# freshman97/LinTransUNet

Hardware: AMD Instinct MI355X
Metric: 128^3 CT patches/sec (fwd+bwd) (higher is better)
Workload: dtype bf16; 1 GPU; MaskTransUnet train step (fwd + 5-level loss + bwd), 128^3 single-channel patches, 2 per GPU, dropout 0.3, random-init weights; global_batch=2, parallelism=dp1, side_stream_concurrent=True, allreduce=none (1 rank)

## Files before the change

### lintransunet_amd/csrc/linattn.hip

```cpp
#include "common.h"

#define DK 32
#define TOK 32
#define PART_STRIDE (64 + 1024)
#ifndef LA_TR_PAD
#define LA_TR_PAD 32
#endif

__device__ __forceinline__ float xhalf_sum(float v) { return xhalf_combine<LtuAdd>(v); }
__device__ __forceinline__ float xhalf_max(float v) { return xhalf_combine<LtuMax>(v); }

__device__ __forceinline__ bf16x8 pack8(const float* v) {
  bf16x8 r;
#pragma unroll
  for (int e = 0; e < 8; ++e) r[e] = (__bf16)v[e];
  return r;
}
template <typename T>
struct IsBf16 { static constexpr bool value = false; };
template <>
struct IsBf16<bf16_t> { static constexpr bool value = true; };

template <typename T>
struct GVec;
template <>
struct GVec<float> {
  static constexpr int W = 4;
  typedef float4 reg;
  static __device__ __forceinline__ reg load(const float* p) { return *reinterpret_cast<const float4*>(p); }
  static __device__ __forceinline__ reg zero() { return make_float4(0.f, 0.f, 0.f, 0.f); }
  static __device__ __forceinline__ void to_lds(float* dst, reg v) { *reinterpret_cast<float4*>(dst) = v; }
  static __device__ __forceinline__ void from_lds(float* gdst, const float* src) {
    *reinterpret_cast<float4*>(gdst) = *reinterpret_cast<const float4*>(src);
  }
  static __device__ __forceinline__ reg pack_lds(const float* src) { return *reinterpret_cast<const float4*>(src); }
  static __device__ __forceinline__ void store_g(float* gdst, reg v) { *reinterpret_cast<float4*>(gdst) = v; }
};
template <>
struct GVec<bf16_t> {
  static constexpr int W = 8;
  typedef uint4 reg;
  static __device__ __forceinline__ reg load(const bf16_t* p) { return *reinterpret_cast<const uint4*>(p); }
  static __device__ __forceinline__ reg zero() { return make_uint4(0u, 0u, 0u, 0u); }
  static __device__ __forceinline__ void to_lds(float* dst, reg v) {
    float4 a, b;
    a.x = __uint_as_float(v.x << 16); a.y = __uint_as_float(v.x & 0xffff0000u);
    a.z = __uint_as_float(v.y << 16); a.w = __uint_as_float(v.y & 0xffff0000u);
    b.x = __uint_as_float(v.z << 16); b.y = __uint_as_float(v.z & 0xffff0000u);
    b.z = __uint_as_float(v.w << 16); b.w = __uint_as_float(v.w & 0xffff0000u);
    *reinterpret_cast<float4*>(dst) = a;
    *reinterpret_cast<float4*>(dst + 4) = b;
  }
  static __device__ __forceinline__ void from_lds(bf16_t* gdst, const float* src) {
    const float4 a = *reinterpret_cast<const float4*>(src), b = *reinterpret_cast<const float4*>(src + 4);
    uint4 v;
    v.x = pack_bf16x2(a.x, a.y);
    v.y = pack_bf16x2(a.z, a.w);
    v.z = pack_bf16x2(b.x, b.y);
    v.w = pack_bf16x2(b.z, b.w);
    *reinterpret_cast<uint4*>(gdst) = v;
  }
  static __device__ __forceinline__ reg pack_lds(const float* src) {
    const float4 a = *reinterpret_cast<const float4*>(src), b = *reinterpret_cast<const float4*>(src + 4);
    return make_uint4(pack_bf16x2(a.x, a.y), pack_bf16x2(a.z, a.w), pack_bf16x2(b.x, b.y), pack_bf16x2(b.z, b.w));
  }
  static __device__ __forceinline__ void store_g(bf16_t* gdst, reg v) { *reinterpret_cast<uint4*>(gdst) = v; }
};

template <typename T, int D, int ROWE, int LDSROW>
struct RowTile {
  static constexpr int NTHR = 2 * D;
  static constexpr int W = GVec<T>::W;
  static constexpr int VPR = ROWE / W;
  static constexpr int NV = (TOK * VPR + NTHR - 1) / NTHR;
  typename GVec<T>::reg r[NV];
  __device__ __forceinline__ void load(const T* gbase, long long gstride, int goff, int n0, int n_end, int tid) {
#pragma unroll
    for (int p = 0; p < NV; ++p) {
      const int idx = tid + p * NTHR;
      const int t = idx / VPR, c = (idx % VPR) * W;
      r[p] = (idx < TOK * VPR && n0 + t < n_end) ? GVec<T>::load(gbase + (long long)(n0 + t) * gstride + goff + c) : GVec<T>::zero();
    }
  }
  __device__ __forceinline__ void store(float* lds, int tid) const {
#pragma unroll
    for (int p = 0; p < NV; ++p) {
      const int idx = tid + p * NTHR;
      const int t = idx / VPR, c = (idx % VPR) * W;
      if (idx < TOK * VPR) GVec<T>::to_lds(lds + t * LDSROW + c, r[p]);
    }
  }
  __device__ __forceinline__ void store_raw(uint16_t* lds, int tid) const {
#pragma unroll
    for (int p = 0; p < NV; ++p) {
      const int idx = tid + p * NTHR;
      const int t = idx / VPR, c = (idx % VPR) * W;
      if (idx < TOK * VPR) *reinterpret_cast<typename GVec<T>::reg*>(lds + t * LDSROW + c) = r[p];
    }
  }
};

typedef __attribute__((ext_vector_type(4))) short la_s16x4;
typedef __attribute__((address_space(3))) la_s16x4 la_lds_s16x4;
__device__ __forceinline__ int tr_lane_offset(int lane, int pitch) {
  const int gq = lane >> 4, tq = (lane >> 2) & 3, tp = lane & 3;
  return (8 * (gq >> 1) + tq) * pitch + 16 * (gq & 1) + 4 * tp;
}
__device__ __forceinline__ bf16x8 tr_frag(const uint16_t* p, int pitch) {
  union { struct { la_s16x4 l, h; } s; bf16x8 v; } u;
  u.s.l = __builtin_amdgcn_ds_read_tr16_b64_v4i16((la_lds_s16x4*)p);
  u.s.h = __builtin_amdgcn_ds_read_tr16_b64_v4i16((la_lds_s16x4*)(p + 4 * pitch));
  return u.v;
}

template <typename T, int D>
__global__ void __launch_bounds__(2 * D) linattn_kv_partial(const T* __restrict__ qkv, float* __restrict__ part, int N,
                                                           int tokens_per_split) {
  constexpr int H = D / DK, ROW = 2 * D;
  constexpr int PITCH = ROW + LA_TR_PAD;
  constexpr int SMEM_FLOATS = IsBf16<T>::value ? (2 * TOK * PITCH) / 2 : TOK * ROW;
  __shared__ __attribute__((aligned(16))) float smem[SMEM_FLOATS];
  const int b = blockIdx.y, sp = blockIdx.x, nsplit = gridDim.x;
  const int tid = threadIdx.x, lane = tid & 63, wave = tid >> 6;
  const int li = lane & 31, lh = lane >> 5;
  const int n_begin = sp * tokens_per_split;
  const int n_end = min(N, n_begin + tokens_per_split);
  const T* base = qkv + (long long)b * N * 3 * D;

  float m_run = -INFINITY, s_run = 0.f;
  f32x16 acc;
#pragma unroll
  for (int r = 0; r < 16; ++r) acc[r] = 0.f;

  if constexpr (IsBf16<T>::value) {
    uint16_t* sm = reinterpret_cast<uint16_t*>(smem);
    RowTile<T, D, ROW, PITCH> tile;
    const int koff = tr_lane_offset(lane, PITCH) + wave * DK, voff = koff + D;
    tile.load(base, 3 * D, D, n_begin, n_end, tid);
    tile.store_raw(sm, tid);
    __syncthreads();
    int buf = 0;
    for (int n0 = n_begin; n0 < n_end; n0 += TOK) {
      const bool more = n0 + TOK < n_end;
      if (more) tile.load(base, 3 * D, D, n0 + TOK, n_end, tid);
      const uint16_t* S = sm + buf * (TOK * PITCH);
      bf16x8 kf[2], vf[2];
#pragma unroll
      for (int u = 0; u < 2; ++u) {
        kf[u] = tr_frag(S + 16 * u * PITCH + koff, PITCH);
        vf[u] = tr_frag(S + 16 * u * PITCH + voff, PITCH);
      }
      const int ntok = min(TOK, n_end - n0);
      float kx[2][8];
      float mt = -INFINITY;
#pragma unroll
      for (int u = 0; u < 2; ++u)
#pragma unroll
        for (int e = 0; e < 8; ++e) {
          kx[u][e] = (float)kf[u][e];
          if (16 * u + 8 * lh + e < ntok) mt = fmaxf(mt, kx[u][e]);
        }
      mt = xhalf_max(mt);
      const float m_new = fmaxf(m_run, mt);
      const float alpha = __expf(m_run - m_new);
      m_run = m_new;
      s_run *= alpha;
#pragma unroll
      for (int r = 0; r < 16; ++r) acc[r] *= alpha;
#pragma unroll
      for (int u = 0; u < 2; ++u) {
        float pe[8];
#pragma unroll
        for (int e = 0; e < 8; ++e) {
          pe[e] = 16 * u + 8 * lh + e < ntok ? __expf(kx[u][e] - m_new) : 0.f;
          s_run += pe[e];
        }
        acc = __builtin_amdgcn_mfma_f32_32x32x16_bf16(vf[u], pack8(pe), acc, 0, 0, 0);
      }
      if (more) tile.store_raw(sm + (buf ^ 1) * (TOK * PITCH), tid);
      __syncthreads();
      buf ^= 1;
    }
  } else {
  RowTile<T, D, ROW, ROW> tile;
  tile.load(base, 3 * D, D, n_begin, n_end, tid);
  for (int n0 = n_begin; n0 < n_end; n0 += TOK) {
    __syncthreads();
    tile.store(smem, tid);
    __syncthreads();
    if (n0 + TOK < n_end) tile.load(base, 3 * D, D, n0 + TOK, n_end, tid);
    const int ntok = min(TOK, n_end - n0);
    const float* ks = smem + wave * DK;
    const float* vs = smem + D + wave * DK;
    float mt = -INFINITY;
#pragma unroll 4
    for (int t = lh; t < TOK; t += 2)
      if (t < ntok) mt = fmaxf(mt, ks[t * ROW + li]);
    mt = xhalf_max(mt);
    const float m_new = fmaxf(m_run, mt);
    const float alpha = __expf(m_run - m_new);
    m_run = m_new;
    s_run *= alpha;
#pragma unroll
    for (int r = 0; r < 16; ++r) acc[r] *= alpha;
    if constexpr (IsBf16<T>::value) {
#pragma unroll
      for (int u = 0; u < 2; ++u) {
        float pe[8], ve[8];
#pragma unroll
        for (int e = 0; e < 8; ++e) {
          const int t = 16 * u + 8 * lh + e;
          pe[e] = 0.f; ve[e] = 0.f;
          if (t < ntok) {
            pe[e] = __expf(ks[t * ROW + li] - m_new);
            ve[e] = vs[t * ROW + li];
          }
          s_run += pe[e];
        }
        acc = __builtin_amdgcn_mfma_f32_32x32x16_bf16(pack8(ve), pack8(pe), acc, 0, 0, 0);
      }
    } else {
#pragma unroll
      for (int t0 = 0; t0 < TOK; t0 += 2) {
        const int t = t0 + lh;
        float p = 0.f, vv = 0.f;
        if (t < ntok) {
          p = __expf(ks[t * ROW + li] - m_new);
          vv = vs[t * ROW + li];
        }
        s_run += p;
        acc = __builtin_amdgcn_mfma_f32_32x32x2f32(vv, p, acc, 0, 0, 0);
      }
    }
  }
  }
  const float s_tot = xhalf_sum(s_run);
  float* out = part + (((long long)b * nsplit + sp) * H + wave) * PART_STRIDE;
  if (lh == 0) {
    out[li] = m_run;
    out[32 + li] = s_tot;
  }
#pragma unroll
  for (int r = 0; r < 16; ++r) {
    const int j = (r & 3) + 8 * (r >> 2) + 4 * lh;
    out[64 + j * 32 + li] = acc[r];
  }
}

#define KVC_GROUP 16
__global__ void __launch_bounds__(1024) linattn_kv_combine(const float* __restrict__ part, int nsplit, int group,
                                                           float* __restrict__ part2, float* __restrict__ stats,
                                                           float* __restrict__ ctx, int H, int final) {
  const int bh = blockIdx.y, b = bh / H, h = bh % H, g = blockIdx.x;
  const int i = threadIdx.x & 31, j = threadIdx.x >> 5;
  const float* p0 = part + ((long long)b * nsplit * H + h) * PART_STRIDE;
  const long long sstride = (long long)H * PART_STRIDE;
  const int s0 = g * group, s1 = min(nsplit, s0 + group);
  float mv[KVC_GROUP];
#pragma unroll
  for (int q = 0; q < KVC_GROUP; ++q) mv[q] = s0 + q < s1 ? p0[(s0 + q) * sstride + i] : -INFINITY;
  float m = mv[0];
#pragma unroll
  for (int q = 1; q < KVC_GROUP; ++q) m = fmaxf(m, mv[q]);
  float sv[KVC_GROUP], av[KVC_GROUP];
#pragma unroll
  for (int q = 0; q < KVC_GROUP; ++q) {
    const float* p = p0 + (s0 + q) * sstride;
    sv[q] = s0 + q < s1 ? p[32 + i] : 0.f;
    av[q] = s0 + q < s1 ? p[64 + j * 32 + i] : 0.f;
  }
  float ssum = 0.f, a = 0.f;
#pragma unroll
  for (int q = 0; q < KVC_GROUP; ++q) {
    const float f = __expf(mv[q] - m);
    ssum += sv[q] * f;
    a += av[q] * f;
  }
  if (final) {
    ctx[(long long)bh * 1024 + i * 32 + j] = a / ssum;
    if (j == 0) {
      stats[bh * 64 + i] = m;
      stats[bh * 64 + 32 + i] = ssum;
    }
  } else {
    float* o = part2 + (((long long)b * gridDim.x + g) * H + h) * PART_STRIDE;
    o[64 + j * 32 + i] = a;
    if (j == 0) {
      o[i] = m;
      o[32 + i] = ssum;
    }
  }
}

template <int NB>
__global__ void __launch_bounds__(256) linattn_kv_combine1(const float* __restrict__ part, int nsplit, float* __restrict__ stats,
                                                           float* __restrict__ ctx, int H) {
  extern __shared__ __attribute__((aligned(16))) float fs[];
  __shared__ float red[8][32];
  __shared__ float4 red4[7][32];
  const int bh = blockIdx.y, b = bh / H, h = bh % H;
  const float* p0 = part + ((long long)b * nsplit * H + h) * PART_STRIDE;
  const long long sstride = (long long)H * PART_STRIDE;
  const int l = threadIdx.x & 31, grp = threadIdx.x >> 5;
  const bool fast = nsplit <= 8 * NB;
  float m = -INFINITY, ss = 0.f;
  const int e0 = blockIdx.x * 128 + l * 4, c0 = e0 & 31;
  float4 a = make_float4(0.f, 0.f, 0.f, 0.f);
  if (fast) {
    float pm[NB], ps[NB];
#pragma unroll
    for (int k = 0; k < NB; ++k) {
      const int sp = grp + 8 * k, sc = sp < nsplit ? sp : 0;
      pm[k] = p0[sc * sstride + l];
      ps[k] = p0[sc * sstride + 32 + l];
    }
#pragma unroll
    for (int k = 0; k < NB; ++k)
      if (grp + 8 * k < nsplit) m = fmaxf(m, pm[k]);
    red[grp][l] = m;
    __syncthreads();
#pragma unroll
    for (int q = 0; q < 8; ++q) m = fmaxf(m, red[q][l]);
    __syncthreads();
    float4 v[NB];
#pragma unroll
    for (int k = 0; k < NB; ++k) {
      const int sp = grp + 8 * k, sc = sp < nsplit ? sp : 0;
      v[k] = *reinterpret_cast<const float4*>(p0 + sc * sstride + 64 + e0);
    }
#pragma unroll
    for (int k = 0; k < NB; ++k) {
      const int sp = grp + 8 * k;
      if (sp < nsplit) {
        const float f = __expf(pm[k] - m);
        fs[sp * 32 + l] = f;
        ss += ps[k] * f;
      }
    }
    red[grp][l] = ss;
    __syncthreads();
    ss = 0.f;
#pragma unroll
    for (int q = 0; q < 8; ++q) ss += red[q][l];
#pragma unroll
    for (int k = 0; k < NB; ++k) {
      const int sp = grp + 8 * k;
      if (sp < nsplit) {
        const float4 f = *reinterpret_cast<const float4*>(fs + sp * 32 + c0);
        a.x += v[k].x * f.x; a.y += v[k].y * f.y; a.z += v[k].z * f.z; a.w += v[k].w * f.w;
      }
    }
  } else {
#pragma unroll 8
    for (int s = grp; s < nsplit; s += 8) m = fmaxf(m, p0[s * sstride + l]);
    red[grp][l] = m;
    __syncthreads();
#pragma unroll
    for (int q = 0; q < 8; ++q) m = fmaxf(m, red[q][l]);
    __syncthreads();
#pragma unroll 8
    for (int s = grp; s < nsplit; s += 8) {
      const float f = __expf(p0[s * sstride + l] - m);
      fs[s * 32 + l] = f;
      ss += p0[s * sstride + 32 + l] * f;
    }
    red[grp][l] = ss;
    __syncthreads();
    ss = 0.f;
#pragma unroll
    for (int q = 0; q < 8; ++q) ss += red[q][l];
#pragma unroll 8
    for (int s = grp; s < nsplit; s += 8) {
      const float4 v = *reinterpret_cast<const float4*>(p0 + s * sstride + 64 + e0);
      const float4 f = *reinterpret_cast<const float4*>(fs + s * 32 + c0);
      a.x += v.x * f.x; a.y += v.y * f.y; a.z += v.z * f.z; a.w += v.w * f.w;
    }
  }
  if (grp > 0) red4[grp - 1][l] = a;
  __shared__ float scol[32];
  if (grp == 0) scol[l] = ss;
  __syncthreads();
  if (grp != 0) return;
#pragma unroll
  for (int q = 0; q < 7; ++q) {
    const float4 v = red4[q][l];
    a.x += v.x; a.y += v.y; a.z += v.z; a.w += v.w;
  }
  const int j = e0 >> 5;
  float* o = ctx + (long long)bh * 1024 + j;
  o[c0 * 32] = a.x / scol[c0]; o[(c0 + 1) * 32] = a.y / scol[c0 + 1]; o[(c0 + 2) * 32] = a.z / scol[c0 + 2]; o[(c0 + 3) * 32] = a.w / scol[c0 + 3];
  if (blockIdx.x == 0) {
    stats[bh * 64 + l] = m;
    stats[bh * 64 + 32 + l] = ss;
  }
}

template <typename T, int D>
__global__ void __launch_bounds__(2 * D) linattn_apply(const T* __restrict__ qkv, const float* __restrict__ ctx, T* __restrict__ out,
                                                      float* __restrict__ qstat, int N, int tokb) {
  constexpr int H = D / DK, LDQ = D + 4, NTHR = 2 * D, W = GVec<T>::W;
  __shared__ __attribute__((aligned(16))) float smem[TOK * LDQ];
  const int b = blockIdx.y;
  const int tid = threadIdx.x, lane = tid & 63, wave = tid >> 6;
  const int li = lane & 31, lh = lane >> 5;
  float cb[16];
  const float* cx = ctx + ((long long)b * H + wave) * 1024;
#pragma unroll
  for (int s = 0; s < 16; ++s) cb[s] = cx[(16 * lh + s) * 32 + li];
  const bf16x8 cbb[2] = {pack8(cb), pack8(cb + 8)};
  const float rs = 0.17677669529663688110f;
  const T* base = qkv + (long long)b * N * 3 * D;

  const int n_begin = blockIdx.x * tokb;
  const int n_end = min(N, n_begin + tokb);
  RowTile<T, D, D, LDQ> tile;
  tile.load(base, 3 * D, 0, n_begin, n_end, tid);
  for (int n0 = n_begin; n0 < n_end; n0 += TOK) {
    __syncthreads();
    tile.store(smem, tid);
    __syncthreads();
    if (n0 + TOK < n_end) tile.load(base, 3 * D, 0, n0 + TOK, n_end, tid);
    float a[16];
    const float* qrow = &smem[li * LDQ + wave * DK + 16 * lh];
#pragma unroll
    for (int q4 = 0; q4 < 4; ++q4) {
      const float4 v = *reinterpret_cast<const float4*>(qrow + 4 * q4);
      a[4 * q4] = v.x; a[4 * q4 + 1] = v.y; a[4 * q4 + 2] = v.z; a[4 * q4 + 3] = v.w;
    }
    float mx = -INFINITY;
#pragma unroll
    for (int s = 0; s < 16; ++s) mx = fmaxf(mx, a[s]);
    mx = xhalf_max(mx);
    float sum = 0.f;
#pragma unroll
    for (int s = 0; s < 16; ++s) {
      a[s] = __expf(a[s] - mx);
      sum += a[s];
    }
    sum = xhalf_sum(sum);
    const float inv = rs / sum;
    if (lh == 0 && n0 + li < n_end) {
      float* qs = qstat + (((long long)b * N + n0 + li) * H + wave) * 2;
      qs[0] = mx;
      qs[1] = inv;
    }
    f32x16 acc;
#pragma unroll
    for (int r = 0; r < 16; ++r) acc[r] = 0.f;
    if constexpr (IsBf16<T>::value) {
#pragma unroll
      for (int s = 0; s < 16; ++s) a[s] *= inv;
      acc = __builtin_amdgcn_mfma_f32_32x32x16_bf16(pack8(a), cbb[0], acc, 0, 0, 0);
      acc = __builtin_amdgcn_mfma_f32_32x32x16_bf16(pack8(a + 8), cbb[1], acc, 0, 0, 0);
    } else {
#pragma unroll
      for (int s = 0; s < 16; ++s) acc = __builtin_amdgcn_mfma_f32_32x32x2f32(a[s] * inv, cb[s], acc, 0, 0, 0);
    }
    __syncthreads();
#pragma unroll
    for (int r = 0; r < 16; ++r) {
      const int t = (r & 3) + 8 * (r >> 2) + 4 * lh;
      smem[t * LDQ + wave * DK + li] = acc[r];
    }
    __syncthreads();
    constexpr int VPR = D / W;
#pragma unroll
    for (int p = 0; p < (TOK * VPR + NTHR - 1) / NTHR; ++p) {
      const int idx = tid + p * NTHR;
      const int t = idx / VPR, c = (idx % VPR) * W;
      if (idx < TOK * VPR && n0 + t < n_end) GVec<T>::from_lds(out + ((long long)b * N + n0 + t) * D + c, &smem[t * LDQ + c]);
    }
  }
}

#define LAW_HEADS 4
#define LAW_LD (LAW_HEADS * DK + 8)

template <int D>
__global__ void __launch_bounds__(256) linattn_apply_rows(const uint16_t* __restrict__ qkv, const float* __restrict__ ctx,
                                                         uint16_t* __restrict__ out, float* __restrict__ qstat, int N, int tiles_per_wave) {
  constexpr int H = D / DK, CG = H / LAW_HEADS;
  __shared__ __attribute__((aligned(16))) uint16_t smem[4 * TOK * LAW_LD];
  const int lane = threadIdx.x & 63, wave = threadIdx.x >> 6;
  const int li = lane & 31, lh = lane >> 5;
  uint16_t* tile = smem + wave * TOK * LAW_LD;
  const int b = blockIdx.y;
  const int gw = blockIdx.x * 4 + wave;
  const int cg = gw % CG;
  const int n_begin = (gw / CG) * tiles_per_wave * TOK;
  const int n_end = min(N, n_begin + tiles_per_wave * TOK);
  if (n_begin >= N) return;
  bf16x8 ca[LAW_HEADS][2];
#pragma unroll
  for (int hh = 0; hh < LAW_HEADS; ++hh) {
    const float* cx = ctx + ((long long)b * H + cg * LAW_HEADS + hh) * 1024;
#pragma unroll
    for (int u = 0; u < 2; ++u) {
      float t[8];
#pragma unroll
      for (int e = 0; e < 8; ++e) t[e] = cx[(16 * lh + 8 * u + e) * 32 + li];
      ca[hh][u] = pack8(t);
    }
  }
  const float rs = 0.17677669529663688110f;
  const int cr = lane >> 4, cc = (lane & 15) * 8;
  const uint16_t* qb = qkv + (long long)b * N * 3 * D + cg * (LAW_HEADS * DK) + cc;
  uint16_t* ob = out + (long long)b * N * D + cg * (LAW_HEADS * DK) + cc;
  uint4 nx[8];
  auto fetch = [&](int n0) {
#pragma unroll
    for (int p = 0; p < 8; ++p) {
      const int n = n0 + 4 * p + cr;
      nx[p] = make_uint4(0u, 0u, 0u, 0u);
      if (n < n_end) nx[p] = *reinterpret_cast<const uint4*>(qb + (long long)n * 3 * D);
    }
  };
  fetch(n_begin);
  for (int n0 = n_begin; n0 < n_end; n0 += TOK) {
#pragma unroll
    for (int p = 0; p < 8; ++p) *reinterpret_cast<uint4*>(tile + (4 * p + cr) * LAW_LD + cc) = nx[p];
    if (n0 + TOK < n_end) fetch(n0 + TOK);
    float2 st[LAW_HEADS];
#pragma unroll
    for (int hh = 0; hh < LAW_HEADS; ++hh) {
      const uint16_t* qr = tile + li * LAW_LD + hh * DK + 16 * lh;
      const uint4 v0 = *reinterpret_cast<const uint4*>(qr), v1 = *reinterpret_cast<const uint4*>(qr + 8);
      const uint32_t w[8] = {v0.x, v0.y, v0.z, v0.w, v1.x, v1.y, v1.z, v1.w};
      float a[16];
#pragma unroll
      for (int k = 0; k < 8; ++k) {
        a[2 * k] = __uint_as_float(w[k] << 16);
        a[2 * k + 1] = __uint_as_float(w[k] & 0xffff0000u);
      }
      float mx = a[0];
#pragma unroll
      for (int s = 1; s < 16; ++s) mx = fmaxf(mx, a[s]);
      mx = xhalf_max(mx);
      float sum = 0.f;
#pragma unroll
      for (int s = 0; s < 16; ++s) {
        a[s] = __expf(a[s] - mx);
        sum += a[s];
      }
      sum = xhalf_sum(sum);
      const float inv = rs / sum;
      st[hh] = make_float2(mx, inv);
#pragma unroll
      for (int s = 0; s < 16; ++s) a[s] *= inv;
      f32x16 acc;
#pragma unroll
      for (int r = 0; r < 16; ++r) acc[r] = 0.f;
      acc = __builtin_amdgcn_mfma_f32_32x32x16_bf16(ca[hh][0], pack8(a), acc, 0, 0, 0);
      acc = __builtin_amdgcn_mfma_f32_32x32x16_bf16(ca[hh][1], pack8(a + 8), acc, 0, 0, 0);
#pragma unroll
      for (int q = 0; q < 4; ++q) {
        uint2 v;
        v.x = pack_bf16x2(acc[4 * q], acc[4 * q + 1]);
        v.y = pack_bf16x2(acc[4 * q + 2], acc[4 * q + 3]);
        *reinterpret_cast<uint2*>(tile + li * LAW_LD + hh * DK + 8 * q + 4 * lh) = v;
      }
    }
    if (lh == 0 && n0 + li < n_end) {
      float4* qs = reinterpret_cast<float4*>(qstat + (((long long)b * N + n0 + li) * H + cg * LAW_HEADS) * 2);
      qs[0] = make_float4(st[0].x, st[0].y, st[1].x, st[1].y);
      qs[1] = make_float4(st[2].x, st[2].y, st[3].x, st[3].y);
    }
#pragma unroll
    for (int p = 0; p < 8; ++p) {
      const int n = n0 + 4 * p + cr;
      const uint4 v = *reinterpret_cast<const uint4*>(tile + (4 * p + cr) * LAW_LD + cc);
      if (n < n_end) *reinterpret_cast<uint4*>(ob + (long long)n * D) = v;
    }
  }
}

template <typename T, int D>
__global__ void __launch_bounds__(2 * D) linattn_dctx_partial(const T* __restrict__ qkv, const T* __restrict__ dout,
                                                             const float* __restrict__ qstat, float* __restrict__ part, int N,
                                                             int tokens_per_split) {
  constexpr int H = D / DK;
  extern __shared__ __attribute__((aligned(16))) float smem[];
  float* sq = smem;
  float* sg = smem + TOK * D;
  float* st = smem + 2 * TOK * D;
  const int b = blockIdx.y, sp = blockIdx.x, nsplit = gridDim.x;
  const int tid = threadIdx.x, lane = tid & 63, wave = tid >> 6;
  const int li = lane & 31, lh = lane >> 5;
  const int n_begin = sp * tokens_per_split;
  const int n_end = min(N, n_begin + tokens_per_split);
  const T* qb = qkv + (long long)b * N * 3 * D;
  const T* gb = dout + (long long)b * N * D;
  f32x16 acc;
#pragma unroll
  for (int r = 0; r < 16; ++r) acc[r] = 0.f;
  RowTile<T, D, D, D> tq, tg;
  static_assert(TOK * H * 2 <= 2 * D, "one statistics float per thread");
  auto load_stat = [&](int n0) {
    return (tid < TOK * H * 2 && n0 + tid / (H * 2) < n_end) ? qstat[((long long)b * N + n0) * H * 2 + tid] : 0.f;
  };
  if constexpr (IsBf16<T>::value) {
    constexpr int PQ = D + LA_TR_PAD;
    uint16_t* sm = reinterpret_cast<uint16_t*>(smem);
    float* stf = reinterpret_cast<float*>(sm + 4 * TOK * PQ);
    RowTile<T, D, D, PQ> bq, bg;
    const int off = tr_lane_offset(lane, PQ) + wave * DK;
    bq.load(qb, 3 * D, 0, n_begin, n_end, tid);
    bg.load(gb, D, 0, n_begin, n_end, tid);
    float stn = load_stat(n_begin);
    bq.store_raw(sm, tid);
    bg.store_raw(sm + TOK * PQ, tid);
    if (tid < TOK * H * 2) stf[tid] = stn;
    __syncthreads();
    int buf = 0;
    for (int n0 = n_begin; n0 < n_end; n0 += TOK) {
      const bool more = n0 + TOK < n_end;
      if (more) {
        bq.load(qb, 3 * D, 0, n0 + TOK, n_end, tid);
        bg.load(gb, D, 0, n0 + TOK, n_end, tid);
        stn = load_stat(n0 + TOK);
      }
      const uint16_t* S = sm + buf * (2 * TOK * PQ);
      const float* ST = stf + buf * (TOK * H * 2);
      const int ntok = min(TOK, n_end - n0);
#pragma unroll
      for (int u = 0; u < 2; ++u) {
        const bf16x8 qf = tr_frag(S + 16 * u * PQ + off, PQ), gf = tr_frag(S + (TOK + 16 * u) * PQ + off, PQ);
        float qe[8];
#pragma unroll
        for (int e = 0; e < 8; ++e) {
          const int t = 16 * u + 8 * lh + e;
          const float2 rs = *reinterpret_cast<const float2*>(ST + (t * H + wave) * 2);
          qe[e] = t < ntok ? __expf((float)qf[e] - rs.x) * rs.y : 0.f;
        }
        acc = __builtin_amdgcn_mfma_f32_32x32x16_bf16(gf, pack8(qe), acc, 0, 0, 0);
      }
      if (more) {
        uint16_t* Sn = sm + (buf ^ 1) * (2 * TOK * PQ);
        bq.store_raw(Sn, tid);
        bg.store_raw(Sn + TOK * PQ, tid);
        if (tid < TOK * H * 2) stf[(buf ^ 1) * (TOK * H * 2) + tid] = stn;
      }
      __syncthreads();
      buf ^= 1;
    }
  } else {
  tq.load(qb, 3 * D, 0, n_begin, n_end, tid);
  tg.load(gb, D, 0, n_begin, n_end, tid);
  float stn = load_stat(n_begin);
  for (int n0 = n_begin; n0 < n_end; n0 += TOK) {
    __syncthreads();
    tq.store(sq, tid);
    tg.store(sg, tid);
    if (tid < TOK * H * 2) st[tid] = stn;
    __syncthreads();
    if (n0 + TOK < n_end) {
      tq.load(qb, 3 * D, 0, n0 + TOK, n_end, tid);
      tg.load(gb, D, 0, n0 + TOK, n_end, tid);
      stn = load_stat(n0 + TOK);
    }
    const int ntok = min(TOK, n_end - n0);
    if constexpr (IsBf16<T>::value) {
#pragma unroll
      for (int u = 0; u < 2; ++u) {
        float qe[8], ge[8];
#pragma unroll
        for (int e = 0; e < 8; ++e) {
          const int t = 16 * u + 8 * lh + e;
          qe[e] = 0.f; ge[e] = 0.f;
          if (t < ntok) {
            qe[e] = __expf(sq[t * D + wave * DK + li] - st[(t * H + wave) * 2]) * st[(t * H + wave) * 2 + 1];
            ge[e] = sg[t * D + wave * DK + li];
          }
        }
        acc = __builtin_amdgcn_mfma_f32_32x32x16_bf16(pack8(ge), pack8(qe), acc, 0, 0, 0);
      }
    } else {
#pragma unroll
      for (int t0 = 0; t0 < TOK; t0 += 2) {
        const int t = t0 + lh;
        float qv = 0.f, gv = 0.f;
        if (t < ntok) {
          qv = __expf(sq[t * D + wave * DK + li] - st[(t * H + wave) * 2]) * st[(t * H + wave) * 2 + 1];
          gv = sg[t * D + wave * DK + li];
        }
        acc = __builtin_amdgcn_mfma_f32_32x32x2f32(gv, qv, acc, 0, 0, 0);
      }
    }
  }
  }
  float* out = part + (((long long)b * nsplit + sp) * H + wave) * 1024;
#pragma unroll
  for (int r = 0; r < 16; ++r) {
    const int j = (r & 3) + 8 * (r >> 2) + 4 * lh;
    out[j * 32 + li] = acc[r];
  }
}

template <int NB>
__global__ void __launch_bounds__(256) linattn_dctx_combine(const float* __restrict__ part, float* __restrict__ dctx, int nsplit, int H) {
  __shared__ float4 red4[7][32];
  const int bh = blockIdx.y, b = bh / H, h = bh % H;
  const float* p0 = part + ((long long)b * nsplit * H + h) * 1024 + blockIdx.x * 128;
  const int l = threadIdx.x & 31, grp = threadIdx.x >> 5;
  float4 a = make_float4(0.f, 0.f, 0.f, 0.f);
  for (int s0 = grp; s0 < nsplit; s0 += 8 * NB) {
    float4 v[NB];
#pragma unroll
    for (int k = 0; k < NB; ++k) {
      const int sp = s0 + 8 * k;
      v[k] = *reinterpret_cast<const float4*>(p0 + (long long)(sp < nsplit ? sp : s0) * H * 1024 + l * 4);
    }
#pragma unroll
    for (int k = 0; k < NB; ++k)
      if (s0 + 8 * k < nsplit) { a.x += v[k].x; a.y += v[k].y; a.z += v[k].z; a.w += v[k].w; }
  }
  if (grp > 0) red4[grp - 1][l] = a;
  __syncthreads();
  if (grp != 0) return;
#pragma unroll
  for (int q = 0; q < 7; ++q) {
    const float4 v = red4[q][l];
    a.x += v.x; a.y += v.y; a.z += v.z; a.w += v.w;
  }
  const int e = blockIdx.x * 128 + l * 4, jj = e >> 5, ii = e & 31;
  float* o = dctx + (long long)bh * 1024 + jj;
  o[ii * 32] = a.x; o[(ii + 1) * 32] = a.y; o[(ii + 2) * 32] = a.z; o[(ii + 3) * 32] = a.w;
}

template <typename T, int D>
__global__ void __launch_bounds__(2 * D, 2) linattn_bwd_apply(const T* __restrict__ qkv, const T* __restrict__ dout,
                                                          const float* __restrict__ ctx, const float* __restrict__ dctx,
                                                          const float* __restrict__ stats, const float* __restrict__ tvec,
                                                          const float* __restrict__ qstat, T* __restrict__ dqkv, int N, int tokb) {
  constexpr int H = D / DK, LD3 = 3 * D + 4, LD1 = D + 4, NTHR = 2 * D, W = GVec<T>::W;
  extern __shared__ __attribute__((aligned(16))) float smem[];
  const int b = blockIdx.y;
  const int tid = threadIdx.x, lane = tid & 63, wave = tid >> 6;
  const int li = lane & 31, lh = lane >> 5;
  float* gt = smem + TOK * LD3;
  float* cs = gt + TOK * LD1 + wave * 96;
  const long long bh = (long long)b * H + wave;
  if (lane < 32) {
    cs[lane] = stats[bh * 64 + lane];
    cs[32 + lane] = 1.f / stats[bh * 64 + 32 + lane];
  }
  float ctxA[16], dcA[16], dcT[16];
#pragma unroll
  for (int s = 0; s < 16; ++s) {
    ctxA[s] = ctx[bh * 1024 + li * 32 + 16 * lh + s];
    dcA[s] = dctx[bh * 1024 + li * 32 + 16 * lh + s];
    dcT[s] = dctx[bh * 1024 + (16 * lh + s) * 32 + li];
  }
  {
    float t = 0.f;
#pragma unroll
    for (int s = 0; s < 16; ++s) t += ctxA[s] * dcA[s];
    t = xhalf_sum(t);
    if (lane < 32) cs[64 + lane] = t;
  }
  const bf16x8 ctxB[2] = {pack8(ctxA), pack8(ctxA + 8)}, dcTB[2] = {pack8(dcT), pack8(dcT + 8)};
  bf16x8 dcAB[3][2];
  {
    float r1[16], r2[16];
#pragma unroll
    for (int s = 0; s < 16; ++s) {
      r1[s] = dcA[s] - (float)(__bf16)dcA[s];
      r2[s] = r1[s] - (float)(__bf16)r1[s];
    }
#pragma unroll
    for (int u = 0; u < 2; ++u) { dcAB[0][u] = pack8(dcA + 8 * u); dcAB[1][u] = pack8(r1 + 8 * u); dcAB[2][u] = pack8(r2 + 8 * u); }
  }
  const T* qb = qkv + (long long)b * N * 3 * D;
  const T* gb = dout + (long long)b * N * D;

  const int n_begin = blockIdx.x * tokb;
  const int n_end = min(N, n_begin + tokb);
  RowTile<T, D, 3 * D, LD3> tq;
  RowTile<T, D, D, LD1> tg;
  auto load_qs = [&](int n0) {
    return *reinterpret_cast<const float2*>(qstat + (((long long)b * N + min(n0 + li, n_end - 1)) * H + wave) * 2);
  };
  tq.load(qb, 3 * D, 0, n_begin, n_end, tid);
  tg.load(gb, D, 0, n_begin, n_end, tid);
  float2 qsn = load_qs(n_begin);
  tq.store(smem, tid);
  tg.store(gt, tid);
  __syncthreads();
  for (int n0 = n_begin; n0 < n_end; n0 += TOK) {
    const float rmax = qsn.x, rinv = qsn.y;
    const bool more = n0 + TOK < n_end;
    if (more) {
      tq.load(qb, 3 * D, 0, n0 + TOK, n_end, tid);
      tg.load(gb, D, 0, n0 + TOK, n_end, tid);
      qsn = load_qs(n0 + TOK);
    }
    const float* qrow = &smem[li * LD3 + wave * DK];
    const float* krow = qrow + D;
    const float* vrow = qrow + 2 * D;
    const float* grow = &gt[li * LD1 + wave * DK];

    float gj[16], kk[16], vj[16];
#pragma unroll
    for (int q4 = 0; q4 < 4; ++q4) {
      const float4 a = *reinterpret_cast<const float4*>(grow + 16 * lh + 4 * q4);
      const float4 c = *reinterpret_cast<const float4*>(krow + 16 * lh + 4 * q4);
      const float4 e = *reinterpret_cast<const float4*>(vrow + 16 * lh + 4 * q4);
      gj[4 * q4] = a.x; gj[4 * q4 + 1] = a.y; gj[4 * q4 + 2] = a.z; gj[4 * q4 + 3] = a.w;
      kk[4 * q4] = c.x; kk[4 * q4 + 1] = c.y; kk[4 * q4 + 2] = c.z; kk[4 * q4 + 3] = c.w;
      vj[4 * q4] = e.x; vj[4 * q4 + 1] = e.y; vj[4 * q4 + 2] = e.z; vj[4 * q4 + 3] = e.w;
    }
    f32x16 aq, av, ak;
#pragma unroll
    for (int r = 0; r < 16; ++r) { aq[r] = 0.f; av[r] = 0.f; ak[r] = 0.f; }
    if constexpr (IsBf16<T>::value) {
#pragma unroll
      for (int s = 0; s < 16; ++s) kk[s] = __expf(kk[s] - cs[16 * lh + s]) * cs[32 + 16 * lh + s];
#pragma unroll
      for (int u = 0; u < 2; ++u) {
        aq = __builtin_amdgcn_mfma_f32_32x32x16_bf16(ctxB[u], pack8(gj + 8 * u), aq, 0, 0, 0);
        av = __builtin_amdgcn_mfma_f32_32x32x16_bf16(dcTB[u], pack8(kk + 8 * u), av, 0, 0, 0);
        const bf16x8 vb = pack8(vj + 8 * u);
#pragma unroll
        for (int pc = 2; pc >= 0; --pc) ak = __builtin_amdgcn_mfma_f32_32x32x16_bf16(dcAB[pc][u], vb, ak, 0, 0, 0);
      }
    } else {
#pragma unroll
      for (int s = 0; s < 16; ++s) {
        const int ch = 16 * lh + s;
        const float pk = __expf(kk[s] - cs[ch]) * cs[32 + ch];
        aq = __builtin_amdgcn_mfma_f32_32x32x2f32(ctxA[s], gj[s], aq, 0, 0, 0);
        av = __builtin_amdgcn_mfma_f32_32x32x2f32(dcT[s], pk, av, 0, 0, 0);
        ak = __builtin_amdgcn_mfma_f32_32x32x2f32(dcA[s], vj[s], ak, 0, 0, 0);
      }
    }
    float dot = 0.f;
    float qsv[16], pkv[16];
#pragma unroll
    for (int g4 = 0; g4 < 4; ++g4) {
      const int i0 = 8 * g4 + 4 * lh;
      const float4 qv = *reinterpret_cast<const float4*>(qrow + i0);
      const float4 kv = *reinterpret_cast<const float4*>(krow + i0);
      const float qa[4] = {qv.x, qv.y, qv.z, qv.w}, ka[4] = {kv.x, kv.y, kv.z, kv.w};
#pragma unroll
      for (int e = 0; e < 4; ++e) {
        const int r = 4 * g4 + e;
        qsv[r] = __expf(qa[e] - rmax) * rinv;
        pkv[r] = __expf(ka[e] - cs[i0 + e]) * cs[32 + i0 + e];
        dot += qsv[r] * aq[r];
      }
    }
    dot = xhalf_sum(dot);
    dot *= 5.65685424949238019521f;
    __syncthreads();
#pragma unroll
    for (int g4 = 0; g4 < 4; ++g4) {
      const int i0 = 8 * g4 + 4 * lh;
      float4 oq, ok4, ov;
#pragma unroll
      for (int e = 0; e < 4; ++e) {
        const int r = 4 * g4 + e;
        f4at(oq, e) = qsv[r] * (aq[r] - dot);
        f4at(ok4, e) = pkv[r] * (ak[r] - cs[64 + i0 + e]);
        f4at(ov, e) = av[r];
      }
      *reinterpret_cast<float4*>(&smem[li * LD3 + wave * DK + i0]) = oq;
      *reinterpret_cast<float4*>(&smem[li * LD3 + D + wave * DK + i0]) = ok4;
      *reinterpret_cast<float4*>(&smem[li * LD3 + 2 * D + wave * DK + i0]) = ov;
    }
    __syncthreads();
    constexpr int VPR = 3 * D / W, NOUT = (TOK * VPR + NTHR - 1) / NTHR;
    typename GVec<T>::reg ovec[NOUT];
#pragma unroll
    for (int p = 0; p < NOUT; ++p) {
      const int idx = min(tid + p * NTHR, TOK * VPR - 1);
      ovec[p] = GVec<T>::pack_lds(&smem[(idx / VPR) * LD3 + (idx % VPR) * W]);
    }
    __syncthreads();
    if (more) {
      tq.store(smem, tid);
      tg.store(gt, tid);
    }
#pragma unroll
    for (int p = 0; p < NOUT; ++p) {
      const int idx = tid + p * NTHR;
      const int t = idx / VPR, c = (idx % VPR) * W;
      if (idx < TOK * VPR && n0 + t < n_end) GVec<T>::store_g(dqkv + ((long long)b * N + n0 + t) * 3 * D + c, ovec[p]);
    }
    __syncthreads();
  }
}

static int pick_splits(int B, int N, int d, int* tokens_per_split) {
  int total = -1;
  total = ltu_knob_pos("LTU_LA_SPLITS", d >= 256 ? 256 : 512);
  int want = total / (B > 0 ? B : 1);
  if (want < 1) want = 1;
  if (want > KVC_GROUP * KVC_GROUP) want = KVC_GROUP * KVC_GROUP;
  int tps = (N + want - 1) / want;
  tps = (tps + 31) / 32 * 32;
  if (tps < 32) tps = 32;
  *tokens_per_split = tps;
  return (N + tps - 1) / tps;
}
static int pick_tokb(int B, int N, int d) {
  const int blocks = ltu_knob_pos("LTU_LA_TOKB_BLOCKS", d <= 128 ? 512 : 256);
  long long per = ((long long)B * N + blocks - 1) / blocks;
  int tokb = (int)((per + 31) / 32 * 32);
  if (tokb < 32) tokb = 32;
  if (tokb > 512) tokb = 512;
  return tokb;
}

extern "C" int ltu_linattn_splits(int B, int N) {
  int tps;
  return pick_splits(B, N, 128, &tps);
}

#define LA_DISPATCH_D(d, ...)                                   \
  do {                                                          \
    if ((d) == 32) { constexpr int D = 32; __VA_ARGS__ }        \
    else if ((d) == 64) { constexpr int D = 64; __VA_ARGS__ }   \
    else if ((d) == 128) { constexpr int D = 128; __VA_ARGS__ } \
    else if ((d) == 256) { constexpr int D = 256; __VA_ARGS__ } \
    else return LTU_E_SHAPE;                                    \
  } while (0)

extern "C" int ltu_linattn_fwd(const void* qkv, void* out, float* ctx, float* colstats, float* qstat, float* part_ws,
                               long long ws_floats, int B, int N, int d, int dtype, ltu_stream_t s);
extern "C" long long ltu_linattn_ws_floats(int B, int N, int d) {
  int tps;
  const long long ns = pick_splits(B, N, d, &tps), H = d / 32;
  return (long long)B * (ns + (ns + KVC_GROUP - 1) / KVC_GROUP + 2) * H * PART_STRIDE;
}
extern "C" int ltu_linattn_ctx(const void* qkv, float* ctx, float* colstats, float* part_ws, long long ws_floats, int B, int N, int d,
                               int dtype, ltu_stream_t s) {
  return ltu_linattn_fwd(qkv, nullptr, ctx, colstats, nullptr, part_ws, ws_floats, B, N, d, dtype, s);
}
extern "C" int ltu_linattn_fwd(const void* qkv, void* out, float* ctx, float* colstats, float* qstat, float* part_ws,
                               long long ws_floats, int B, int N, int d, int dtype, ltu_stream_t s) {
  const int H = d / 32;
  int tps;
  const int nsplit = pick_splits(B, N, d, &tps);
  if ((long long)B * (nsplit + (nsplit + KVC_GROUP - 1) / KVC_GROUP + 2) * H * PART_STRIDE > ws_floats) return LTU_E_ARG;
  hipStream_t st = (hipStream_t)s;
  const int tokb = pick_tokb(B, N, d);
  LTU_DISPATCH_T(dtype, {
    LA_DISPATCH_D(d, {
      hipLaunchKernelGGL((linattn_kv_partial<T, D>), dim3(nsplit, B), dim3(2 * D), 0, st, (const T*)qkv, part_ws, N, tps);
      const int group = KVC_GROUP, ngroups = (nsplit + group - 1) / group;
      float* part2 = part_ws + (size_t)B * nsplit * H * PART_STRIDE;
      if (nsplit * 32 * sizeof(float) <= 48 * 1024 && !ltu_knob("LTU_LA_TWO_LEVEL", 0)) {
        const size_t fsb = (size_t)nsplit * 32 * sizeof(float);
        if (nsplit <= 32) hipLaunchKernelGGL(linattn_kv_combine1<4>, dim3(8, B * H), dim3(256), fsb, st, part_ws, nsplit, colstats, ctx, H);
        else if (nsplit <= 64) hipLaunchKernelGGL(linattn_kv_combine1<8>, dim3(8, B * H), dim3(256), fsb, st, part_ws, nsplit, colstats, ctx, H);
        else if (nsplit <= 128) hipLaunchKernelGGL(linattn_kv_combine1<16>, dim3(8, B * H), dim3(256), fsb, st, part_ws, nsplit, colstats, ctx, H);
        else hipLaunchKernelGGL(linattn_kv_combine1<32>, dim3(8, B * H), dim3(256), fsb, st, part_ws, nsplit, colstats, ctx, H);
      } else if (ngroups > 1) {
        hipLaunchKernelGGL(linattn_kv_combine, dim3(ngroups, B * H), dim3(1024), 0, st, part_ws, nsplit, group, part2, colstats, ctx, H, 0);
        hipLaunchKernelGGL(linattn_kv_combine, dim3(1, B * H), dim3(1024), 0, st, part2, ngroups, ngroups, nullptr, colstats, ctx, H, 1);
      } else {
        hipLaunchKernelGGL(linattn_kv_combine, dim3(1, B * H), dim3(1024), 0, st, part_ws, nsplit, nsplit, nullptr, colstats, ctx, H, 1);
      }
      if (out == nullptr) {
      } else if constexpr (IsBf16<T>::value && D >= 128) {
        constexpr int CG = D / DK / LAW_HEADS;
        const long long tiles = cdiv(N, TOK);
        long long tpw = cdiv((long long)B * tiles * CG, (long long)ltu_knob_pos("LTU_LA_APPLY_WAVES", 4096));
        if (tpw < 1) tpw = 1;
        const long long waves = cdiv(tiles, tpw) * CG;
        hipLaunchKernelGGL((linattn_apply_rows<D>), dim3((unsigned)cdiv(waves, 4), B), dim3(256), 0, st, (const uint16_t*)qkv, ctx, (uint16_t*)out, qstat, N, (int)tpw);
      } else {
        hipLaunchKernelGGL((linattn_apply<T, D>), dim3(cdiv(N, tokb), B), dim3(2 * D), 0, st, (const T*)qkv, ctx, (T*)out, qstat, N, tokb);
      }
    });
  });
  return ltu_check_launch();
}

extern "C" int ltu_linattn_bwd(const void* qkv, const void* dout, const float* ctx, const float* colstats,
                               const float* qstat, void* dqkv, float* dctx, float* tvec, float* part_ws, long long ws_floats, int B,
                               int N, int d, int dtype, ltu_stream_t s) {
  const int H = d / 32;
  int tps;
  const int nsplit = pick_splits(B, N, d, &tps);
  if ((long long)B * nsplit * H * 1024 > ws_floats) return LTU_E_ARG;
  hipStream_t st = (hipStream_t)s;
  const size_t lds_b = (size_t)(32 * (3 * d + 4) + 32 * (d + 4) + H * 96) * sizeof(float);
  const int tokb = pick_tokb(B, N, d);
  LTU_DISPATCH_T(dtype, {
    LA_DISPATCH_D(d, {
      const size_t lds_p = IsBf16<T>::value ? (size_t)4 * TOK * (D + LA_TR_PAD) * 2 + (size_t)2 * TOK * H * 2 * sizeof(float)
                                            : (size_t)(2 * TOK * D + TOK * H * 2) * sizeof(float);
      hipLaunchKernelGGL((linattn_dctx_partial<T, D>), dim3(nsplit, B), dim3(2 * D), lds_p, st, (const T*)qkv, (const T*)dout, qstat, part_ws, N, tps);
      if (nsplit <= 32) hipLaunchKernelGGL(linattn_dctx_combine<4>, dim3(8, B * H), dim3(256), 0, st, part_ws, dctx, nsplit, H);
      else if (nsplit <= 64) hipLaunchKernelGGL(linattn_dctx_combine<8>, dim3(8, B * H), dim3(256), 0, st, part_ws, dctx, nsplit, H);
      else if (nsplit <= 128) hipLaunchKernelGGL(linattn_dctx_combine<16>, dim3(8, B * H), dim3(256), 0, st, part_ws, dctx, nsplit, H);
      else hipLaunchKernelGGL(linattn_dctx_combine<32>, dim3(8, B * H), dim3(256), 0, st, part_ws, dctx, nsplit, H);
      hipLaunchKernelGGL((linattn_bwd_apply<T, D>), dim3(cdiv(N, tokb), B), dim3(2 * D), lds_b, st, (const T*)qkv, (const T*)dout, ctx, dctx, colstats, tvec, qstat, (T*)dqkv, N, tokb);
    });
  });
  return ltu_check_launch();
}
```

Baseline: 161.5 patches/s.

## Fuse dQ into dctx partial pass and split linear-attention bwd by head groups

For bf16 and D>=128, the dQ gradient is now computed inside the dctx partial kernel, which reuses the already-staged q and dout tiles and flushes results to dqkv. The apply kernel then only computes dK and dV. It uses 256-thread blocks over two-head column groups with per-wave token ranges, and keeps dctx as a three-term bf16 split to preserve precision in the MFMA. This removes a separate full reread of q and dout, improves occupancy and wave-level parallelism, and replaces the wide per-block LDS tile. The risks are extra work and register pressure in the partial kernel, plus more complex ordering of writes to dqkv.

```diff
diff --git a/lintransunet_amd/csrc/linattn.hip b/lintransunet_amd/csrc/linattn.hip
--- a/lintransunet_amd/csrc/linattn.hip
+++ b/lintransunet_amd/csrc/linattn.hip
@@ -575,10 +575,17 @@
 }
 
 template <typename T, int D>
-__global__ void __launch_bounds__(2 * D) linattn_dctx_partial(const T* __restrict__ qkv, const T* __restrict__ dout,
-                                                             const float* __restrict__ qstat, float* __restrict__ part, int N,
+struct LaSplitBwd { static constexpr bool value = IsBf16<T>::value && D >= 128; };
+
+#define LA_P1_WAVES(T, D) (LaSplitBwd<T, D>::value ? 4 : 1)
+
+template <typename T, int D>
+__global__ void __launch_bounds__(2 * D, LA_P1_WAVES(T, D)) linattn_dctx_partial(const T* __restrict__ qkv, const T* __restrict__ dout,
+                                                             const float* __restrict__ qstat, const float* __restrict__ ctx,
+                                                             float* __restrict__ part, T* __restrict__ dqkv, int N,
                                                              int tokens_per_split) {
   constexpr int H = D / DK;
+  constexpr bool DQ = LaSplitBwd<T, D>::value;
   extern __shared__ __attribute__((aligned(16))) float smem[];
   float* sq = smem;
   float* sg = smem + TOK * D;
@@ -610,6 +617,25 @@
     bq.store_raw(sm, tid);
     bg.store_raw(sm + TOK * PQ, tid);
     if (tid < TOK * H * 2) stf[tid] = stn;
+    bf16x8 ctxB[2];
+    if constexpr (DQ) {
+      const float* cx = ctx + ((long long)b * H + wave) * 1024 + li * 32 + 16 * lh;
+      float ctxA[16];
+#pragma unroll
+      for (int s = 0; s < 16; ++s) ctxA[s] = cx[s];
+      ctxB[0] = pack8(ctxA);
+      ctxB[1] = pack8(ctxA + 8);
+    }
+    auto flush_dq = [&](const uint16_t* S, int n) {
+      constexpr int VPR = D / 8;
+#pragma unroll
+      for (int p = 0; p < RowTile<T, D, D, PQ>::NV; ++p) {
+        const int idx = tid + p * RowTile<T, D, D, PQ>::NTHR;
+        const int t = idx / VPR, c = (idx % VPR) * 8;
+        const uint4 v = *reinterpret_cast<const uint4*>(S + t * PQ + c);
+        if (idx < TOK * VPR && n + t < n_end) *reinterpret_cast<uint4*>(dqkv + ((long long)b * N + n + t) * 3 * D + c) = v;
+      }
+    };
     __syncthreads();
     int buf = 0;
     for (int n0 = n_begin; n0 < n_end; n0 += TOK) {
@@ -619,7 +645,10 @@
         bg.load(gb, D, 0, n0 + TOK, n_end, tid);
         stn = load_stat(n0 + TOK);
       }
-      const uint16_t* S = sm + buf * (2 * TOK * PQ);
+      if constexpr (DQ) {
+        if (n0 > n_begin) flush_dq(sm + (buf ^ 1) * (2 * TOK * PQ), n0 - TOK);
+      }
+      uint16_t* S = sm + buf * (2 * TOK * PQ);
       const float* ST = stf + buf * (TOK * H * 2);
       const int ntok = min(TOK, n_end - n0);
 #pragma unroll
@@ -633,6 +662,45 @@
           qe[e] = t < ntok ? __expf((float)qf[e] - rs.x) * rs.y : 0.f;
         }
         acc = __builtin_amdgcn_mfma_f32_32x32x16_bf16(gf, pack8(qe), acc, 0, 0, 0);
+      }
+      if constexpr (DQ) {
+        uint16_t* qrow = S + li * PQ + wave * DK;
+        const uint16_t* grow = S + (TOK + li) * PQ + wave * DK + 16 * lh;
+        f32x16 aq;
+#pragma unroll
+        for (int r = 0; r < 16; ++r) aq[r] = 0.f;
+#pragma unroll
+        for (int u = 0; u < 2; ++u) {
+          union { uint4 r; bf16x8 v; } gj;
+          gj.r = *reinterpret_cast<const uint4*>(grow + 8 * u);
+          aq = __builtin_amdgcn_mfma_f32_32x32x16_bf16(ctxB[u], gj.v, aq, 0, 0, 0);
+        }
+        const float2 rq = *reinterpret_cast<const float2*>(ST + (li * H + wave) * 2);
+        const float rmax = rq.x, rinv = rq.y;
+        float dot = 0.f;
+        float qsv[16];
+#pragma unroll
+        for (int g4 = 0; g4 < 4; ++g4) {
+          const uint2 qv = *reinterpret_cast<const uint2*>(qrow + 8 * g4 + 4 * lh);
+          const float qa[4] = {__uint_as_float(qv.x << 16), __uint_as_float(qv.x & 0xffff0000u), __uint_as_float(qv.y << 16),
+                               __uint_as_float(qv.y & 0xffff0000u)};
+#pragma unroll
+          for (int e = 0; e < 4; ++e) {
+            const int r = 4 * g4 + e;
+            qsv[r] = __expf(qa[e] - rmax) * rinv;
+            dot += qsv[r] * aq[r];
+          }
+        }
+        dot = xhalf_sum(dot);
+        dot *= 5.65685424949238019521f;
+        __builtin_amdgcn_fence(__ATOMIC_ACQ_REL, "wavefront");
+#pragma unroll
+        for (int g4 = 0; g4 < 4; ++g4) {
+          uint2 o;
+          o.x = pack_bf16x2(qsv[4 * g4] * (aq[4 * g4] - dot), qsv[4 * g4 + 1] * (aq[4 * g4 + 1] - dot));
+          o.y = pack_bf16x2(qsv[4 * g4 + 2] * (aq[4 * g4 + 2] - dot), qsv[4 * g4 + 3] * (aq[4 * g4 + 3] - dot));
+          *reinterpret_cast<uint2*>(qrow + 8 * g4 + 4 * lh) = o;
+        }
       }
       if (more) {
         uint16_t* Sn = sm + (buf ^ 1) * (2 * TOK * PQ);
@@ -643,6 +711,7 @@
       __syncthreads();
       buf ^= 1;
     }
+    if constexpr (DQ) flush_dq(sm + (buf ^ 1) * (2 * TOK * PQ), n_begin + (n_end - n_begin - 1) / TOK * TOK);
   } else {
   tq.load(qb, 3 * D, 0, n_begin, n_end, tid);
   tg.load(gb, D, 0, n_begin, n_end, tid);
@@ -727,13 +796,185 @@
   o[ii * 32] = a.x; o[(ii + 1) * 32] = a.y; o[(ii + 2) * 32] = a.z; o[(ii + 3) * 32] = a.w;
 }
 
+#define LAB_HEADS 2
+#define LAB_KV (LAB_HEADS * DK)
+#define LAB_LD (2 * LAB_KV + 8)
+#define LAB_MLD 36
+
+#define LA_P2_WAVES(T, D) (LaSplitBwd<T, D>::value ? 3 : 2)
+
 template <typename T, int D>
-__global__ void __launch_bounds__(2 * D, 2) linattn_bwd_apply(const T* __restrict__ qkv, const T* __restrict__ dout,
-                                                          const float* __restrict__ ctx, const float* __restrict__ dctx,
-                                                          const float* __restrict__ stats, const float* __restrict__ tvec,
-                                                          const float* __restrict__ qstat, T* __restrict__ dqkv, int N, int tokb) {
+__global__ void __launch_bounds__(2 * D, LA_P2_WAVES(T, D))
+linattn_bwd_apply(const T* __restrict__ qkv, const T* __restrict__ dout, const float* __restrict__ ctx, const float* __restrict__ dctx,
+                  const float* __restrict__ stats, float* __restrict__ tvec, const float* __restrict__ qstat, T* __restrict__ dqkv,
+                  int N, int tokb) {
+  extern __shared__ __attribute__((aligned(16))) float smem[];
+  if constexpr (LaSplitBwd<T, D>::value) {
+    constexpr int H = D / DK, CG = H / LAB_HEADS;
+    static_assert(4 * TOK * LAB_LD * 2 >= 2 * LAB_HEADS * 32 * LAB_MLD * 4, "the staged matrices fit the tile space");
+    const int tid = threadIdx.x, lane = tid & 63, wave = tid >> 6;
+    const int li = lane & 31, lh = lane >> 5;
+    const int b = blockIdx.y, cg = blockIdx.x % CG, chunk = blockIdx.x / CG;
+    const long long bh0 = (long long)b * H + cg * LAB_HEADS;
+    uint16_t* tile = reinterpret_cast<uint16_t*>(smem) + wave * TOK * LAB_LD;
+    float* cs = smem + 4 * TOK * LAB_LD / 2;
+    float* mat = smem;
+    static_assert(LAB_HEADS == 2, "staging maps below");
+#pragma unroll
+    for (int p = 0; p < 4; ++p) {
+      const float* src = (p < 2 ? ctx : dctx) + (bh0 + (p & 1)) * 1024;
+      *reinterpret_cast<float4*>(mat + p * 32 * LAB_MLD + (tid >> 3) * LAB_MLD + (tid & 7) * 4) =
+          *reinterpret_cast<const float4*>(src + tid * 4);
+    }
+    if (tid < 128) {
+      const int hh = tid >> 6;
+      const float v = stats[(bh0 + hh) * 64 + lane];
+      cs[hh * 96 + lane] = lane < 32 ? v : 1.f / v;
+    }
+    __syncthreads();
+    bf16x8 dcTB[LAB_HEADS][2], dcAB[LAB_HEADS][3][2];
+#pragma unroll
+    for (int hh = 0; hh < LAB_HEADS; ++hh) {
+      const float* mc = mat + hh * 32 * LAB_MLD;
+      const float* md = mat + (2 + hh) * 32 * LAB_MLD;
+      float ctxA[16], dcA[16], dcT[16];
+#pragma unroll
+      for (int q4 = 0; q4 < 4; ++q4) {
+        const float4 a = *reinterpret_cast<const float4*>(mc + li * LAB_MLD + 16 * lh + 4 * q4);
+        const float4 c = *reinterpret_cast<const float4*>(md + li * LAB_MLD + 16 * lh + 4 * q4);
+        ctxA[4 * q4] = a.x; ctxA[4 * q4 + 1] = a.y; ctxA[4 * q4 + 2] = a.z; ctxA[4 * q4 + 3] = a.w;
+        dcA[4 * q4] = c.x; dcA[4 * q4 + 1] = c.y; dcA[4 * q4 + 2] = c.z; dcA[4 * q4 + 3] = c.w;
+      }
+#pragma unroll
+      for (int s = 0; s < 16; ++s) dcT[s] = md[(16 * lh + s) * LAB_MLD + li];
+      float t = 0.f;
+#pragma unroll
+      for (int s = 0; s < 16; ++s) t += ctxA[s] * dcA[s];
+      t = xhalf_sum(t);
+      if (wave == 0 && lane < 32) {
+        cs[hh * 96 + 64 + lane] = t;
+        if (tvec != nullptr && chunk == 0) tvec[(bh0 + hh) * 32 + lane] = t;
+      }
+      dcTB[hh][0] = pack8(dcT);
+      dcTB[hh][1] = pack8(dcT + 8);
+      float r1[16], r2[16];
+#pragma unroll
+      for (int s = 0; s < 16; ++s) {
+        r1[s] = dcA[s] - (float)(__bf16)dcA[s];
+        r2[s] = r1[s] - (float)(__bf16)r1[s];
+      }
+#pragma unroll
+      for (int u = 0; u < 2; ++u) {
+        dcAB[hh][0][u] = pack8(dcA + 8 * u);
+        dcAB[hh][1][u] = pack8(r1 + 8 * u);
+        dcAB[hh][2][u] = pack8(r2 + 8 * u);
+      }
+    }
+    __syncthreads();
+    const int n_begin = (chunk * 4 + wave) * tokb * TOK;
+    const int n_end = (int)min((long long)N, (long long)n_begin + (long long)tokb * TOK);
+    const int cr = lane >> 3, cc = (lane & 7) * 8;
+    const uint16_t* kb = reinterpret_cast<const uint16_t*>(qkv) + (long long)b * N * 3 * D + D + cg * LAB_KV + cc;
+    uint16_t* ob = reinterpret_cast<uint16_t*>(dqkv) + (long long)b * N * 3 * D + D + cg * LAB_KV + cc;
+    uint4 nk[4], nv[4];
+    auto fetch = [&](int n0) {
+#pragma unroll
+      for (int p = 0; p < 4; ++p) {
+        const int n = n0 + 8 * p + cr;
+        nk[p] = make_uint4(0u, 0u, 0u, 0u);
+        nv[p] = make_uint4(0u, 0u, 0u, 0u);
+        if (n < n_end) {
+          nk[p] = *reinterpret_cast<const uint4*>(kb + (long long)n * 3 * D);
+          nv[p] = *reinterpret_cast<const uint4*>(kb + (long long)n * 3 * D + D);
+        }
+      }
+    };
+    auto stage = [&]() {
+#pragma unroll
+      for (int p = 0; p < 4; ++p) {
+        *reinterpret_cast<uint4*>(tile + (8 * p + cr) * LAB_LD + cc) = nk[p];
+        *reinterpret_cast<uint4*>(tile + (8 * p + cr) * LAB_LD + LAB_KV + cc) = nv[p];
+      }
+    };
+    if (n_begin < n_end) {
+      fetch(n_begin);
+      stage();
+    }
+    for (int n0 = n_begin; n0 < n_end; n0 += TOK) {
+      const bool more = n0 + TOK < n_end;
+      if (more) fetch(n0 + TOK);
+#pragma unroll
+      for (int hh = 0; hh < LAB_HEADS; ++hh) {
+        uint16_t* krow = tile + li * LAB_LD + hh * DK;
+        uint16_t* vrow = krow + LAB_KV;
+        const float* ch = cs + hh * 96;
+        const uint4 k0 = *reinterpret_cast<const uint4*>(krow + 16 * lh), k1 = *reinterpret_cast<const uint4*>(krow + 16 * lh + 8);
+        union { uint4 r; bf16x8 v; } vb[2];
+        vb[0].r = *reinterpret_cast<const uint4*>(vrow + 16 * lh);
+        vb[1].r = *reinterpret_cast<const uint4*>(vrow + 16 * lh + 8);
+        const uint32_t kw[8] = {k0.x, k0.y, k0.z, k0.w, k1.x, k1.y, k1.z, k1.w};
+        float kk[16];
+#pragma unroll
+        for (int k = 0; k < 8; ++k) {
+          kk[2 * k] = __uint_as_float(kw[k] << 16);
+          kk[2 * k + 1] = __uint_as_float(kw[k] & 0xffff0000u);
+        }
+#pragma unroll
+        for (int s = 0; s < 16; ++s) kk[s] = __expf(kk[s] - ch[16 * lh + s]) * ch[32 + 16 * lh + s];
+        f32x16 av, ak;
+#pragma unroll
+        for (int r = 0; r < 16; ++r) { av[r] = 0.f; ak[r] = 0.f; }
+#pragma unroll
+        for (int u = 0; u < 2; ++u) {
+          av = __builtin_amdgcn_mfma_f32_32x32x16_bf16(dcTB[hh][u], pack8(kk + 8 * u), av, 0, 0, 0);
+#pragma unroll
+          for (int pc = 2; pc >= 0; --pc) ak = __builtin_amdgcn_mfma_f32_32x32x16_bf16(dcAB[hh][pc][u], vb[u].v, ak, 0, 0, 0);
+        }
+        float pkv[16];
+#pragma unroll
+        for (int g4 = 0; g4 < 4; ++g4) {
+          const int i0 = 8 * g4 + 4 * lh;
+          const uint2 kv = *reinterpret_cast<const uint2*>(krow + i0);
+          const float ka[4] = {__uint_as_float(kv.x << 16), __uint_as_float(kv.x & 0xffff0000u), __uint_as_float(kv.y << 16),
+                               __uint_as_float(kv.y & 0xffff0000u)};
+#pragma unroll
+          for (int e = 0; e < 4; ++e) pkv[4 * g4 + e] = __expf(ka[e] - ch[i0 + e]) * ch[32 + i0 + e];
+        }
+        __builtin_amdgcn_fence(__ATOMIC_ACQ_REL, "wavefront");
+#pragma unroll
+        for (int g4 = 0; g4 < 4; ++g4) {
+          const int i0 = 8 * g4 + 4 * lh;
+          float dk4[4];
+#pragma unroll
+          for (int e = 0; e < 4; ++e) dk4[e] = pkv[4 * g4 + e] * (ak[4 * g4 + e] - ch[64 + i0 + e]);
+          uint2 o;
+          o.x = pack_bf16x2(dk4[0], dk4[1]);
+          o.y = pack_bf16x2(dk4[2], dk4[3]);
+          *reinterpret_cast<uint2*>(krow + i0) = o;
+          o.x = pack_bf16x2(av[4 * g4], av[4 * g4 + 1]);
+          o.y = pack_bf16x2(av[4 * g4 + 2], av[4 * g4 + 3]);
+          *reinterpret_cast<uint2*>(vrow + i0) = o;
+        }
+      }
+      __builtin_amdgcn_fence(__ATOMIC_ACQ_REL, "wavefront");
+      uint4 ok[4], ov[4];
+#pragma unroll
+      for (int p = 0; p < 4; ++p) {
+        ok[p] = *reinterpret_cast<const uint4*>(tile + (8 * p + cr) * LAB_LD + cc);
+        ov[p] = *reinterpret_cast<const uint4*>(tile + (8 * p + cr) * LAB_LD + LAB_KV + cc);
+      }
+      if (more) stage();
+#pragma unroll
+      for (int p = 0; p < 4; ++p) {
+        const int n = n0 + 8 * p + cr;
+        if (n < n_end) {
+          *reinterpret_cast<uint4*>(ob + (long long)n * 3 * D) = ok[p];
+          *reinterpret_cast<uint4*>(ob + (long long)n * 3 * D + D) = ov[p];
+        }
+      }
+    }
+  } else {
   constexpr int H = D / DK, LD3 = 3 * D + 4, LD1 = D + 4, NTHR = 2 * D, W = GVec<T>::W;
-  extern __shared__ __attribute__((aligned(16))) float smem[];
   const int b = blockIdx.y;
   const int tid = threadIdx.x, lane = tid & 63, wave = tid >> 6;
   const int li = lane & 31, lh = lane >> 5;
@@ -887,6 +1128,7 @@
       if (idx < TOK * VPR && n0 + t < n_end) GVec<T>::store_g(dqkv + ((long long)b * N + n0 + t) * 3 * D + c, ovec[p]);
     }
     __syncthreads();
+  }
   }
 }
 
@@ -985,18 +1227,27 @@
   const int nsplit = pick_splits(B, N, d, &tps);
   if ((long long)B * nsplit * H * 1024 > ws_floats) return LTU_E_ARG;
   hipStream_t st = (hipStream_t)s;
-  const size_t lds_b = (size_t)(32 * (3 * d + 4) + 32 * (d + 4) + H * 96) * sizeof(float);
   const int tokb = pick_tokb(B, N, d);
   LTU_DISPATCH_T(dtype, {
     LA_DISPATCH_D(d, {
       const size_t lds_p = IsBf16<T>::value ? (size_t)4 * TOK * (D + LA_TR_PAD) * 2 + (size_t)2 * TOK * H * 2 * sizeof(float)
                                             : (size_t)(2 * TOK * D + TOK * H * 2) * sizeof(float);
-      hipLaunchKernelGGL((linattn_dctx_partial<T, D>), dim3(nsplit, B), dim3(2 * D), lds_p, st, (const T*)qkv, (const T*)dout, qstat, part_ws, N, tps);
+      hipLaunchKernelGGL((linattn_dctx_partial<T, D>), dim3(nsplit, B), dim3(2 * D), lds_p, st, (const T*)qkv, (const T*)dout, qstat, ctx, part_ws, (T*)dqkv, N, tps);
       if (nsplit <= 32) hipLaunchKernelGGL(linattn_dctx_combine<4>, dim3(8, B * H), dim3(256), 0, st, part_ws, dctx, nsplit, H);
       else if (nsplit <= 64) hipLaunchKernelGGL(linattn_dctx_combine<8>, dim3(8, B * H), dim3(256), 0, st, part_ws, dctx, nsplit, H);
       else if (nsplit <= 128) hipLaunchKernelGGL(linattn_dctx_combine<16>, dim3(8, B * H), dim3(256), 0, st, part_ws, dctx, nsplit, H);
       else hipLaunchKernelGGL(linattn_dctx_combine<32>, dim3(8, B * H), dim3(256), 0, st, part_ws, dctx, nsplit, H);
-      hipLaunchKernelGGL((linattn_bwd_apply<T, D>), dim3(cdiv(N, tokb), B), dim3(2 * D), lds_b, st, (const T*)qkv, (const T*)dout, ctx, dctx, colstats, tvec, qstat, (T*)dqkv, N, tokb);
+      if constexpr (LaSplitBwd<T, D>::value) {
+        constexpr int CG = D / DK / LAB_HEADS;
+        const size_t lds_b = (size_t)4 * TOK * LAB_LD * 2 + (size_t)LAB_HEADS * 96 * sizeof(float);
+        const long long tiles = cdiv(N, TOK);
+        long long tpw = cdiv((long long)B * tiles * CG, (long long)ltu_knob_pos("LTU_LA_BWD_WAVES", 2048));
+        if (tpw < 1) tpw = 1;
+        hipLaunchKernelGGL((linattn_bwd_apply<T, D>), dim3(cdiv(tiles, 4 * tpw) * CG, B), dim3(256), lds_b, st, (const T*)qkv, (const T*)dout, ctx, dctx, colstats, tvec, qstat, (T*)dqkv, N, (int)tpw);
+      } else {
+        const size_t lds_b = (size_t)(32 * (3 * d + 4) + 32 * (d + 4) + H * 96) * sizeof(float);
+        hipLaunchKernelGGL((linattn_bwd_apply<T, D>), dim3(cdiv(N, tokb), B), dim3(2 * D), lds_b, st, (const T*)qkv, (const T*)dout, ctx, dctx, colstats, tvec, qstat, (T*)dqkv, N, tokb);
+      }
     });
   });
   return ltu_check_launch();
```

Result: no change. 160.0 patches/s (-1.0%).
